# Xiaoming-Zhao/PointNav-VO

Measured on AMD Instinct MI355X. Metric: RGB-D frame-pair VO inferences/s @341x192, higher is better.
Workload: dtype f32

## Files before the change

### pointnav-vo_amd/csrc/conv_x3.hip

```cpp
#include <cmath>
#include <cstdio>
#include <cstdlib>
#include <cstring>

#include "pnvo_internal.h"

namespace pnvo {

typedef float f32x16 __attribute__((ext_vector_type(16)));
typedef float f32x4 __attribute__((ext_vector_type(4)));
typedef float f32x2 __attribute__((ext_vector_type(2)));
typedef __bf16 bf16x8 __attribute__((ext_vector_type(8)));
typedef __bf16 bf16x2 __attribute__((ext_vector_type(2)));
typedef _Float16 f16x8 __attribute__((ext_vector_type(8)));
typedef _Float16 f16x2 __attribute__((ext_vector_type(2)));
typedef unsigned u32x4 __attribute__((ext_vector_type(4)));

namespace {
__device__ __forceinline__ unsigned pack2(float a, float b) {
  const bf16x2 r = __builtin_convertvector(f32x2{a, b}, bf16x2);
  return __builtin_bit_cast(unsigned, r);
}
__device__ __forceinline__ unsigned pack2h(float a, float b) {
  const f16x2 r = __builtin_convertvector(f32x2{a, b}, f16x2);
  return __builtin_bit_cast(unsigned, r);
}
__device__ __forceinline__ float lo_f(unsigned u) { return __builtin_bit_cast(float, u << 16); }
__device__ __forceinline__ float hi_f(unsigned u) { return __builtin_bit_cast(float, u & 0xffff0000u); }
}

constexpr int x3_wpe(int mw, int nw, int np, bool dsf = false) {
  return dsf ? (mw * nw >= 6 ? 1 : (mw * nw >= 2 ? 2 : 3)) : ((np == 2 && mw * nw <= 2) ? 3 : 2);
}

template <int KS, int STRIDE, int MODE, int MW, int NW, int NP, bool DSF = false, bool W8 = false, bool KSW = false>
__global__ __launch_bounds__(W8 ? 512 : 256) __attribute__((amdgpu_waves_per_eu(W8 ? 2 : x3_wpe(MW, NW, NP, DSF), W8 ? 2 : x3_wpe(MW, NW, NP, DSF)))) void conv_x3_kernel(const ConvX3Args p) {
  constexpr int NTH = W8 ? 512 : 256, NWV = NTH / 64;
  constexpr int EMW = KSW ? 1 : MW;
  static_assert(!KSW || (NW == 1 && NP == 2 && KS == 3 && !DSF && !W8), "K split over the waves: float16-piece 3x3 convs, one N-tile");
  static_assert(!DSF || (KS == 3 && STRIDE == 2 && NP == 2 && (MODE == 0 || MODE == 2)), "the downsample rides on a float16-piece 3x3 stride-2 conv");
  extern __shared__ __attribute__((aligned(16))) unsigned char lds[];
  constexpr int PSTEP = KS == 1 ? STRIDE : 1;
  constexpr int CS = KS == 1 ? 1 : STRIDE;
  constexpr int PAD = KS / 2;
  const int lane = threadIdx.x & 63;
  const int wave = __builtin_amdgcn_readfirstlane(threadIdx.x >> 6);

  const int ntiles = p.B * p.tiles_r * p.tiles_c;
  const int chunk = (ntiles + 7) >> 3;
  int bid = (int)(blockIdx.x & 7) * chunk + (int)(blockIdx.x >> 3);
  if (bid >= ntiles) return;
  const int tci = bid % p.tiles_c;
  bid /= p.tiles_c;
  const int tri = bid % p.tiles_r;
  const int n = bid / p.tiles_r;
  const int r0 = tri * p.TR, c0 = tci * p.TC;
  const int hi0 = r0 * STRIDE - PAD, wi0 = c0 * STRIDE - PAD;
  const int mdl = (p.grp_end0 > 0 && n >= p.grp_end0) + (p.grp_end1 > 0 && n >= p.grp_end1);
  const unsigned short *g_wpk = mdl == 0 ? p.wpk : p.wpk_g[mdl - 1];
  const unsigned short *g_ds_wpk = mdl == 0 ? p.ds_wpk : p.ds_wpk_g[mdl - 1];
  const float g_oscale = mdl == 0 ? p.oscale : p.oscale_g[mdl - 1], g_ds_oscale = mdl == 0 ? p.ds_oscale : p.ds_oscale_g[mdl - 1];
  const float *g_gamma = mdl == 0 ? p.gn_gamma : p.gn_gamma_g[mdl - 1], *g_beta = mdl == 0 ? p.gn_beta : p.gn_beta_g[mdl - 1];
  const float *g_ds_gamma = mdl == 0 ? p.ds_gamma : p.ds_gamma_g[mdl - 1], *g_ds_beta = mdl == 0 ? p.ds_beta : p.ds_beta_g[mdl - 1];
  const int PR = p.PR, PC = p.PC, CK = p.CK;
  const int pitch = CK * 2 + 16;
  const int plane = PR * PC * pitch;
  const int npix = p.TR * p.TC;
  const int tab_off = KSW ? max(NP * plane, 4 * MW * 4096) : NP * plane;
  unsigned *qtab = reinterpret_cast<unsigned *>(lds + tab_off);
  unsigned *otab = qtab + p.MT * 32;
  for (int e = (int)threadIdx.x; e < p.MT * 32; e += NTH) {
    const int q = min(e, npix - 1);
    const int tr = q / p.TC, tc = q - tr * p.TC;
    qtab[e] = (unsigned)(((tr * CS) * PC + tc * CS) * pitch);
    const bool ok = e < npix && r0 + tr < p.Ho && c0 + tc < p.Wo;
    otab[e] = (unsigned)((tr * p.Wo + tc) * p.COUTP) | (ok ? 0u : 0x80000000u);
  }

  const int wn = p.wn;
  const int wave_m = wave / wn;
  const int wave_n = (wave & (wn - 1)) + (int)blockIdx.y * wn;
  const int ntt = p.COUTP >> 5, kct = p.CIN >> 4;

  f32x16 acc[MW][NW];
#pragma unroll
  for (int i = 0; i < MW; ++i)
#pragma unroll
    for (int j = 0; j < NW; ++j)
#pragma unroll
      for (int r = 0; r < 16; ++r) acc[i][j][r] = 0.f;
  f32x16 accd[DSF ? MW : 1][DSF ? NW : 1];
  if (DSF) {
#pragma unroll
    for (int i = 0; i < MW; ++i)
#pragma unroll
      for (int j = 0; j < NW; ++j)
#pragma unroll
        for (int r = 0; r < 16; ++r) accd[DSF ? i : 0][DSF ? j : 0][r] = 0.f;
  }

  float in_mul = 1.f, in_div = 1.f;
  const bool in_scaled = NP == 2 && p.in_absmax != nullptr;
  if (in_scaled) {
    unsigned mb = p.in_absmax[(threadIdx.x & 63) * 16];
#pragma unroll
    for (int d = 32; d >= 1; d >>= 1) mb = max(mb, (unsigned)__shfl_xor((int)mb, d));
    const int e = mb != 0u ? (int)((mb >> 23) & 0xffu) - 126 : 14;
    in_mul = __builtin_bit_cast(float, (unsigned)(14 - e + 127) << 23);
    in_div = __builtin_bit_cast(float, (unsigned)(e - 14 + 127) << 23);
  }
  const int G = CK >> 3;
  const int cg = threadIdx.x & (G - 1), pl = threadIdx.x / G, PS = NTH / G;
  const int dr = PS / PC, dc = PS - dr * PC;
  const int nppix = PR * PC;

  unsigned long long c_stage = 0, c_mm = 0, t_0 = __builtin_readcyclecounter(), r_0 = wall_clock64();
  for (int ck0 = 0; ck0 < p.CIN; ck0 += CK) {
    unsigned long long t_a = __builtin_readcyclecounter();
    if (ck0 > 0) __syncthreads();
    {
      f32x4 sc0, sc1, sh0, sh1, rs0, rs1, rt0, rt1;
      const bool res_ss = MODE == 2 && p.res_scale != nullptr;
      auto load_ss = [&]() {
        if (MODE >= 1) {
          const float *ps = p.in_scale + (long)n * p.CIN + ck0 + 8 * cg;
          const float *pt = p.in_shift + (long)n * p.CIN + ck0 + 8 * cg;
          sc0 = *reinterpret_cast<const f32x4 *>(ps);
          sc1 = *reinterpret_cast<const f32x4 *>(ps + 4);
          sh0 = *reinterpret_cast<const f32x4 *>(pt);
          sh1 = *reinterpret_cast<const f32x4 *>(pt + 4);
        }
        if (res_ss) {
          const float *ps = p.res_scale + (long)n * p.CIN + ck0 + 8 * cg;
          const float *pt = p.res_shift + (long)n * p.CIN + ck0 + 8 * cg;
          rs0 = *reinterpret_cast<const f32x4 *>(ps);
          rs1 = *reinterpret_cast<const f32x4 *>(ps + 4);
          rt0 = *reinterpret_cast<const f32x4 *>(pt);
          rt1 = *reinterpret_cast<const f32x4 *>(pt + 4);
        }
      };
      load_ss();
      int pr = pl / PC, pc = pl - pr * PC;
      const long img = ((long)n * p.H * p.W) * p.CIN + ck0 + 8 * cg;
      const float *xb = p.x + img;
      struct Round {
        f32x4 v[2][2], w[2][2];
        unsigned off[2];
        int gofs[2];
        bool ok[2], in[2], own[2];
      };
      auto fetch = [&](int pix, Round &r) {
#pragma unroll
        for (int k = 0; k < 2; ++k) {
          const int hi = hi0 + pr * PSTEP, wi = wi0 + pc * PSTEP;
          r.ok[k] = pix + k * PS < nppix;
          r.in[k] = r.ok[k] && hi >= 0 && hi < p.H && wi >= 0 && wi < p.W;
          r.off[k] = (unsigned)((pr * PC + pc) * pitch + 16 * cg);
          r.v[k][0] = r.v[k][1] = f32x4{0.f, 0.f, 0.f, 0.f};
          if (MODE >= 2) {
            r.own[k] = r.in[k] && p.xout != nullptr && blockIdx.y == 0 && pr >= PAD && pr < PAD + p.TR * CS && pc >= PAD && pc < PAD + p.TC * CS;
            r.gofs[k] = (hi * p.W + wi) * p.CIN;
          }
          if (r.in[k]) {
            const float *src = xb + ((long)hi * p.W + wi) * p.CIN;
            r.v[k][0] = *reinterpret_cast<const f32x4 *>(src);
            r.v[k][1] = *reinterpret_cast<const f32x4 *>(src + 4);
            if (MODE == 2) {
              const float *rsrc = p.res + img + ((long)hi * p.W + wi) * p.CIN;
              r.w[k][0] = *reinterpret_cast<const f32x4 *>(rsrc);
              r.w[k][1] = *reinterpret_cast<const f32x4 *>(rsrc + 4);
            }
          }
          pr += dr;
          pc += dc;
          if (pc >= PC) {
            pc -= PC;
            pr += 1;
          }
        }
      };
      auto split_store = [&](const Round &r) {
#pragma unroll
        for (int k = 0; k < 2; ++k) {
          if (!r.ok[k]) continue;
          float f[8];
#pragma unroll
          for (int e = 0; e < 8; ++e) {
            float t = r.v[k][e >> 2][e & 3];
            if (MODE == 1) {
              const f32x4 &sc = e < 4 ? sc0 : sc1, &sh = e < 4 ? sh0 : sh1;
              t = r.in[k] ? fmaxf(__builtin_fmaf(t, sc[e & 3], sh[e & 3]), 0.f) : 0.f;
            }
            if (MODE == 3) {
              const f32x4 &sc = e < 4 ? sc0 : sc1, &sh = e < 4 ? sh0 : sh1;
              int key = __builtin_bit_cast(int, t);
              key = key >= 0 ? key : key ^ 0x7fffffff;
              t = r.in[k] ? fmaxf(__builtin_fmaf(__builtin_bit_cast(float, key), __builtin_fabsf(sc[e & 3]), sh[e & 3]), 0.f) : 0.f;
            }
            if (MODE == 2) {
              const f32x4 &sc = e < 4 ? sc0 : sc1, &sh = e < 4 ? sh0 : sh1;
              float u = r.w[k][e >> 2][e & 3];
              if (res_ss) u = __builtin_fmaf(u, (e < 4 ? rs0 : rs1)[e & 3], (e < 4 ? rt0 : rt1)[e & 3]);
              t = r.in[k] ? fmaxf(__builtin_fmaf(t, sc[e & 3], sh[e & 3]) + u, 0.f) : 0.f;
            }
            f[e] = t;
          }
          if (MODE >= 2 && r.own[k]) {
            float *dst = p.xout + img + r.gofs[k];
            *reinterpret_cast<f32x4 *>(dst) = f32x4{f[0], f[1], f[2], f[3]};
            *reinterpret_cast<f32x4 *>(dst + 4) = f32x4{f[4], f[5], f[6], f[7]};
          }
          if (NP == 2) {
            if (in_scaled) {
#pragma unroll
              for (int e = 0; e < 8; ++e) f[e] *= in_mul;
            }
            u32x4 o0, o1;
#pragma unroll
            for (int e = 0; e < 4; ++e) {
              const float a = f[2 * e], b = f[2 * e + 1];
              const f16x2 h = __builtin_convertvector(f32x2{a, b}, f16x2);
              o0[e] = __builtin_bit_cast(unsigned, h);
              o1[e] = pack2h(a - (float)h[0], b - (float)h[1]);
            }
            *reinterpret_cast<u32x4 *>(lds + r.off[k]) = o0;
            *reinterpret_cast<u32x4 *>(lds + plane + r.off[k]) = o1;
            continue;
          }
          u32x4 o0, o1, o2;
#pragma unroll
          for (int e = 0; e < 4; ++e) {
            const float a = f[2 * e], b = f[2 * e + 1];
            const unsigned h = pack2(a, b);
            const float ra = a - lo_f(h), rb = b - hi_f(h);
            const unsigned m = pack2(ra, rb);
            o0[e] = h;
            o1[e] = m;
            o2[e] = pack2(ra - lo_f(m), rb - hi_f(m));
          }
          *reinterpret_cast<u32x4 *>(lds + r.off[k]) = o0;
          *reinterpret_cast<u32x4 *>(lds + plane + r.off[k]) = o1;
          *reinterpret_cast<u32x4 *>(lds + 2 * plane + r.off[k]) = o2;
        }
      };
      constexpr bool PIPE = !((MODE == 2 && (MW * NW >= 6 || x3_wpe(MW, NW, NP) == 3 || DSF)) || (DSF && MW * NW == 4));
      if (MW * NW <= 2 && !(MODE == 2 && (x3_wpe(MW, NW, NP) == 3 || DSF))) {
        for (int pix = pl; pix < nppix; pix += 6 * PS) {
          Round r0, r1, r2;
          fetch(pix, r0);
          fetch(pix + 2 * PS, r1);
          fetch(pix + 4 * PS, r2);
          split_store(r0);
          split_store(r1);
          split_store(r2);
        }
      } else if (PIPE) {
        Round cur, nxt;
        fetch(pl, cur);
        for (int pix = pl; pix < nppix; pix += 2 * PS) {
          const bool more = pix + 2 * PS < nppix;
          if (more) fetch(pix + 2 * PS, nxt);
          split_store(cur);
          if (more) cur = nxt;
        }
      } else {
        for (int pix = pl; pix < nppix; pix += 2 * PS) {
          Round cur;
          fetch(pix, cur);
          split_store(cur);
        }
      }
    }
    __syncthreads();
    unsigned long long t_b = __builtin_readcyclecounter();
    c_stage += t_b - t_a;

    unsigned aoff[MW];
#pragma unroll
    for (int i = 0; i < MW; ++i) {
      const int mt = min(KSW ? i : wave_m * MW + i, p.MT - 1);
      aoff[i] = qtab[mt * 32 + (lane & 31)] + (unsigned)((lane >> 5) * 16);
    }
    const int kcc = CK >> 4;
    const int nsteps = KS * KS * kcc;
    const unsigned kstep = (unsigned)ntt * (NP * 1024u);
    const char *wb_n = reinterpret_cast<const char *>(g_wpk) + (long)(ck0 >> 4) * kstep;
    unsigned toff_n = 0;
    int kc_n = 0, kw_n = 0;
    auto advance = [&]() {
      ++kc_n;
      toff_n += 32;
      wb_n += kstep;
      if (kc_n == kcc) {
        kc_n = 0;
        toff_n += (unsigned)(pitch - kcc * 32);
        wb_n += (long)(kct - kcc) * kstep;
        if (++kw_n == KS) {
          kw_n = 0;
          toff_n += (unsigned)((PC - KS) * pitch);
        }
      }
    };
    constexpr bool RING = NP == 2 && KS == 3 && MW * NW <= 2;
    const char *wb_b = wb_n;
    int kc_b = 0;
    auto advanceB = [&]() {
      wb_b += kstep;
      if (++kc_b == kcc) {
        kc_b = 0;
        wb_b += (long)(kct - kcc) * kstep;
      }
    };
    unsigned voff[NW];
#pragma unroll
    for (int j = 0; j < NW; ++j) voff[j] = (unsigned)min(wave_n * NW + j, ntt - 1) * (NP * 1024u) + (unsigned)lane * 16u;
    auto loadBr = [&](u32x4 (*b)[NW]) {
#pragma unroll
      for (int j = 0; j < NW; ++j)
#pragma unroll
        for (int pc = 0; pc < NP; ++pc) b[pc][j] = *reinterpret_cast<const u32x4 *>(wb_b + (size_t)voff[j] + pc * 1024);
    };
    auto loadA = [&](int i, u32x4 (*a)[MW]) {
#pragma unroll
      for (int pc = 0; pc < NP; ++pc) a[pc][i] = *reinterpret_cast<const u32x4 *>(lds + pc * plane + aoff[i] + toff_n);
    };
    auto loadB = [&](u32x4 (*b)[NW]) {
#pragma unroll
      for (int j = 0; j < NW; ++j)
#pragma unroll
        for (int pc = 0; pc < NP; ++pc) b[pc][j] = *reinterpret_cast<const u32x4 *>(wb_n + (size_t)voff[j] + pc * 1024);
    };
    auto step = [&](u32x4 (*a)[MW], const u32x4 (*b)[NW]) {
#pragma unroll
      for (int i = 0; i < MW; ++i) {
#pragma unroll
        for (int j = 0; j < NW; ++j) {
          if (NP == 2) {
            constexpr int TA[3] = {1, 0, 0}, TB[3] = {0, 1, 0};
#pragma unroll
            for (int t = 0; t < 3; ++t)
              acc[i][j] = __builtin_amdgcn_mfma_f32_32x32x16_f16(__builtin_bit_cast(f16x8, a[TA[t]][i]),
                                                                 __builtin_bit_cast(f16x8, b[TB[t]][j]), acc[i][j], 0, 0, 0);
          } else {
            constexpr int TA[6] = {1, 2, 0, 1, 0, 0}, TB[6] = {1, 0, 2, 0, 1, 0};
#pragma unroll
            for (int t = 0; t < 6; ++t)
              acc[i][j] = __builtin_amdgcn_mfma_f32_32x32x16_bf16(__builtin_bit_cast(bf16x8, a[TA[t]][i]),
                                                                  __builtin_bit_cast(bf16x8, b[TB[t]][j]), acc[i][j], 0, 0, 0);
          }
        }
        __builtin_amdgcn_sched_barrier(0);
        loadA(i, a);
        __builtin_amdgcn_sched_barrier(0);
      }
    };
    u32x4 a[NP][MW], b0[NP][NW], b1[NP][NW];
    u32x4 bd0[DSF ? NP : 1][NW], bd1[DSF ? NP : 1][NW];
    auto loadBd = [&](u32x4 (*b)[NW], int kc) {
      const char *wd = reinterpret_cast<const char *>(g_ds_wpk) + (long)((ck0 >> 4) + kc) * kstep;
#pragma unroll
      for (int j = 0; j < NW; ++j)
#pragma unroll
        for (int pc = 0; pc < NP; ++pc) b[pc][j] = *reinterpret_cast<const u32x4 *>(wd + (size_t)voff[j] + pc * 1024);
    };
    if constexpr (KSW) {
      const int s0 = (wave * nsteps) >> 2, s1 = ((wave + 1) * nsteps) >> 2;
      {
        const int tap = s0 / kcc, kc = s0 - tap * kcc, kh = tap / KS, kw = tap - kh * KS;
        kc_n = kc;
        kw_n = kw;
        toff_n = (unsigned)((kh * PC + kw) * pitch + kc * 32);
        wb_n += ((long)tap * kct + kc) * kstep;
        kc_b = kc;
        wb_b = wb_n;
      }
      u32x4 br[3][NP][NW];
      int fb = s0;
      auto fetchB = [&](u32x4 (*bq)[NW]) {
        loadBr(bq);
        if (++fb < s1) advanceB();
      };
      fetchB(br[0]);
      fetchB(br[1]);
#pragma unroll
      for (int i = 0; i < MW; ++i) loadA(i, a);
      if (s0 + 1 < s1) advance();
#pragma unroll 1
      for (int s = s0; s < s1; s += 3) {
#pragma unroll
        for (int u = 0; u < 3; ++u) {
          if (s + u >= s1) break;
          fetchB(br[(u + 2) % 3]);
          __builtin_amdgcn_sched_barrier(0);
          step(a, br[u]);
          if (s + u + 2 < s1) advance();
        }
      }
    } else {
    if (DSF) loadBd(bd0, 0);
    loadB(b0);
#pragma unroll
    for (int i = 0; i < MW; ++i) loadA(i, a);
    advance();
    if (RING) {
      constexpr int R = MW * NW <= 2 ? 6 : 3;
      u32x4 br[R][NP][NW];
#pragma unroll
      for (int pc = 0; pc < NP; ++pc)
#pragma unroll
        for (int j = 0; j < NW; ++j) br[0][pc][j] = b0[pc][j];
#pragma unroll
      for (int q = 1; q < R - 1; ++q) {
        advanceB();
        loadBr(br[q]);
      }
      advanceB();
      constexpr bool A2 = MW * NW <= 2 && !(MODE == 2 && MW * NW == 2 && !DSF) && !(MODE == 2 && DSF && MW * NW == 1);
      u32x4 a1[A2 ? NP : 1][MW];
      if (A2) {
#pragma unroll
        for (int i = 0; i < MW; ++i) loadA(i, a1);
        advance();
      }
#pragma unroll 1
      for (int s = 0; s < nsteps; s += R) {
#pragma unroll
        for (int u = 0; u < R; ++u) {
          loadBr(br[(u + R - 1) % R]);
          if (s + u + R < nsteps) advanceB();
          __builtin_amdgcn_sched_barrier(0);
          if (A2) {
            step((u & 1) ? a1 : a, br[u]);
            if (s + u + 3 < nsteps) advance();
          } else {
            step(a, br[u]);
            if (s + u + 2 < nsteps) advance();
          }
        }
      }
    } else {
#pragma unroll 1
      for (int s = 0; s < nsteps; s += 2) {
        const bool more = s + 2 < nsteps;
        loadB(b1);
        __builtin_amdgcn_sched_barrier(0);
        step(a, b0);
        if (more) advance();
        loadB(b0);
        __builtin_amdgcn_sched_barrier(0);
        step(a, b1);
        if (more) advance();
      }
    }
    }
    if constexpr (DSF) {
      const unsigned tc0 = (unsigned)((PC + 1) * pitch);
      u32x4 ad[NP][MW];
      auto loadAd = [&](int kc) {
#pragma unroll
        for (int i = 0; i < MW; ++i)
#pragma unroll
          for (int pc = 0; pc < NP; ++pc) ad[pc][i] = *reinterpret_cast<const u32x4 *>(lds + pc * plane + aoff[i] + tc0 + (unsigned)kc * 32u);
      };
      auto mm = [&](const u32x4 (*bd)[NW]) {
        constexpr int TA[3] = {1, 0, 0}, TB[3] = {0, 1, 0};
#pragma unroll
        for (int i = 0; i < MW; ++i)
#pragma unroll
          for (int j = 0; j < NW; ++j)
#pragma unroll
            for (int t = 0; t < 3; ++t)
              accd[i][j] = __builtin_amdgcn_mfma_f32_32x32x16_f16(__builtin_bit_cast(f16x8, ad[TA[t]][i]), __builtin_bit_cast(f16x8, bd[TB[t]][j]),
                                                                  accd[i][j], 0, 0, 0);
      };
      if constexpr (MW * NW == 4) {
#pragma unroll 1
        for (int kc = 0; kc < kcc; ++kc) {
          loadAd(kc);
          mm(bd0);
          if (kc + 1 < kcc) loadBd(bd0, kc + 1);
        }
      } else {
#pragma unroll 1
        for (int kc = 0; kc < kcc; kc += 2) {
          loadAd(kc);
          loadBd(bd1, kc + 1);
          mm(bd0);
          loadAd(kc + 1);
          if (kc + 2 < kcc) loadBd(bd0, kc + 2);
          mm(bd1);
        }
      }
    }
    c_mm += __builtin_readcyclecounter() - t_b;
  }
  if constexpr (KSW) {
    __syncthreads();
    float *part = reinterpret_cast<float *>(lds);
#pragma unroll
    for (int i = 0; i < MW; ++i)
#pragma unroll
      for (int r = 0; r < 16; ++r) part[((wave * MW + i) * 16 + r) * 64 + lane] = acc[i][0][r];
    __syncthreads();
    const int mt = min(wave, MW - 1);
#pragma unroll
    for (int r = 0; r < 16; ++r) {
      float v = part[((0 * MW + mt) * 16 + r) * 64 + lane];
#pragma unroll
      for (int w = 1; w < 4; ++w) v += part[((w * MW + mt) * 16 + r) * 64 + lane];
      acc[0][0][r] = v;
    }
    __syncthreads();
  }
  unsigned long long t_e = __builtin_readcyclecounter();

  const int rr16 = lane >> 5;
  const long ybase = (((long)n * p.Ho + r0) * p.Wo + c0) * p.COUTP;
  auto emit = [&](f32x16 (*ac)[NW], float *yout, float *stats, const float *oscale_ptr, float oscale, const float *gamma, const float *beta,
                  float *gscale, float *gshift, float *gmu, float *grstd, bool again) {
    if (NP == 2) {
      const float os = (oscale_ptr != nullptr ? *oscale_ptr : oscale) * in_div;
#pragma unroll
      for (int i = 0; i < EMW; ++i)
#pragma unroll
        for (int j = 0; j < NW; ++j)
#pragma unroll
          for (int r = 0; r < 16; ++r) ac[i][j][r] *= os;
    }
    float t1[NW], t2[NW];
#pragma unroll
    for (int j = 0; j < NW; ++j) t1[j] = t2[j] = 0.f;
#pragma unroll
    for (int i = 0; i < EMW; ++i) {
      const int mt = KSW ? wave : wave_m * MW + i;
      if (mt >= p.MT) continue;
      u32x4 ent[4];
#pragma unroll
      for (int g4 = 0; g4 < 4; ++g4) ent[g4] = *reinterpret_cast<const u32x4 *>(otab + mt * 32 + 8 * g4 + 4 * rr16);
      unsigned flags = 0;
#pragma unroll
      for (int g4 = 0; g4 < 4; ++g4) flags |= ent[g4][0] | ent[g4][1] | ent[g4][2] | ent[g4][3];
      const bool whole = !__any((int)(flags >> 31));
#pragma unroll
      for (int j = 0; j < NW; ++j) {
        const int nt = wave_n * NW + j;
        if (nt >= ntt) continue;
        const int co = nt * 32 + (lane & 31);
        float s1 = 0.f, s2 = 0.f;
        if (whole) {
#pragma unroll
          for (int r = 0; r < 16; ++r) {
            const float v = ac[i][j][r];
            (yout + ybase + co)[ent[r >> 2][r & 3]] = v;
            s1 += v;
            s2 = __builtin_fmaf(v, v, s2);
          }
        } else {
#pragma unroll
          for (int r = 0; r < 16; ++r) {
            const unsigned e = ent[r >> 2][r & 3];
            const bool ok = (int)e >= 0;
            const float v = ok ? ac[i][j][r] : 0.f;
            if (ok) (yout + ybase + co)[e] = v;
            s1 += v;
            s2 = __builtin_fmaf(v, v, s2);
          }
        }
        t1[j] += s1 + __shfl_xor(s1, 32);
        t2[j] += s2 + __shfl_xor(s2, 32);
      }
    }
    if (stats != nullptr) {
      const int rows = NWV / wn;
      float *red = reinterpret_cast<float *>(lds);
      if (rows > 1) {
        __syncthreads();
        if (lane < 32)
// ... 315 lines not shown
#pragma unroll
          for (int r = 0; r < 16; ++r) acc[i][j][r] *= os;
    }
    const int rr16 = lane >> 5;
    const long ybase = (((long)cur.n * p.Ho + cur.r0) * p.Wo + cur.c0) * p.COUTP;
    float t1[NW], t2[NW];
#pragma unroll
    for (int j = 0; j < NW; ++j) t1[j] = t2[j] = 0.f;
#pragma unroll
    for (int i = 0; i < MW; ++i) {
      const int mt = wave_m * MW + i;
      if (mt >= p.MT) continue;
      u32x4 ent[4];
#pragma unroll
      for (int g4 = 0; g4 < 4; ++g4) ent[g4] = *reinterpret_cast<const u32x4 *>(otab + mt * 32 + 8 * g4 + 4 * rr16);
      unsigned flags = 0;
#pragma unroll
      for (int g4 = 0; g4 < 4; ++g4) flags |= ent[g4][0] | ent[g4][1] | ent[g4][2] | ent[g4][3];
      const bool whole = !__any((int)(flags >> 31));
#pragma unroll
      for (int j = 0; j < NW; ++j) {
        const int nt = wave_n * NW + j;
        if (nt >= ntt) continue;
        const int co = nt * 32 + (lane & 31);
        float s1 = 0.f, s2 = 0.f;
        if (whole) {
#pragma unroll
          for (int r = 0; r < 16; ++r) {
            const float x = acc[i][j][r];
            (p.y + ybase + co)[ent[r >> 2][r & 3]] = x;
            s1 += x;
            s2 = __builtin_fmaf(x, x, s2);
          }
        } else {
#pragma unroll
          for (int r = 0; r < 16; ++r) {
            const unsigned e = ent[r >> 2][r & 3];
            const bool ok = (int)e >= 0;
            const float x = ok ? acc[i][j][r] : 0.f;
            if (ok) (p.y + ybase + co)[e] = x;
            s1 += x;
            s2 = __builtin_fmaf(x, x, s2);
          }
        }
        t1[j] += s1 + __shfl_xor(s1, 32);
        t2[j] += s2 + __shfl_xor(s2, 32);
      }
    }
    if (p.stats != nullptr) {
      const int rows = 4 / wn;
      float *red = reinterpret_cast<float *>(lds);
      if (rows > 1) {
        __syncthreads();
        if (lane < 32)
#pragma unroll
          for (int j = 0; j < NW; ++j) *reinterpret_cast<f32x2 *>(red + ((wave * NW + j) * 32 + lane) * 2) = f32x2{t1[j], t2[j]};
        __syncthreads();
      }
      if (wave_m == 0 && lane < 32) {
#pragma unroll
        for (int j = 0; j < NW; ++j) {
          const int nt = wave_n * NW + j;
          if (nt >= ntt) continue;
          float s1 = t1[j], s2 = t2[j];
          for (int w = 1; w < rows; ++w) {
            const f32x2 o = *reinterpret_cast<const f32x2 *>(red + (((w * wn + (wave & (wn - 1))) * NW + j) * 32 + lane) * 2);
            s1 += o[0];
            s2 += o[1];
          }
          float *dst = p.stats + (((long)cur.n * p.slots + cur.tri * p.tiles_c + cur.tci) * p.COUTP + nt * 32 + lane) * 2;
          dst[0] = s1;
          dst[1] = s2;
        }
      }
    }
    if (!nxt.valid) break;
    if (BRES) fetch(nxt);
    __syncthreads();
    cur = nxt;
  }
}

namespace {
template <int KS, int STRIDE, int NP>
hipError_t launch_ks(const ConvX3Args &a, int mode, int mw, int nw, dim3 grid, size_t ldsb, hipStream_t s) {
#define PNVO_X3(MODE_, MW_, NW_)                                                                          \
  if (mode == MODE_ && mw == MW_ && nw == NW_) {                                                          \
    hipLaunchKernelGGL((conv_x3_kernel<KS, STRIDE, MODE_, MW_, NW_, NP>), grid, dim3(256), ldsb, s, a);   \
    return hipGetLastError();                                                                             \
  }
  if constexpr (KS == 3 && STRIDE == 2 && NP == 2) {
    if (a.ds_wpk != nullptr) {
#define PNVO_X3D(MODE_, MW_, NW_)                                                                               \
  if (mode == MODE_ && mw == MW_ && nw == NW_) {                                                                \
    hipLaunchKernelGGL((conv_x3_kernel<KS, STRIDE, MODE_, MW_, NW_, NP, true>), grid, dim3(256), ldsb, s, a);   \
    return hipGetLastError();                                                                                   \
  }
      if (a.w8) {
#define PNVO_X3DW(MODE_)                                                                                                  \
  if (mode == MODE_ && mw == 3 && nw == 1) {                                                                             \
    hipLaunchKernelGGL((conv_x3_kernel<KS, STRIDE, MODE_, 3, 1, NP, true, true>), grid, dim3(512), ldsb, s, a);          \
    return hipGetLastError();                                                                                            \
  }
        PNVO_X3DW(0) PNVO_X3DW(2)
#undef PNVO_X3DW
        return hipErrorInvalidValue;
      }
      PNVO_X3D(0, 1, 1) PNVO_X3D(2, 1, 1) PNVO_X3D(0, 2, 1) PNVO_X3D(2, 2, 1) PNVO_X3D(0, 2, 2) PNVO_X3D(2, 2, 2) PNVO_X3D(0, 3, 2) PNVO_X3D(2, 3, 2)
#undef PNVO_X3D
      return hipErrorInvalidValue;
    }
  }
  PNVO_X3(0, 1, 1) PNVO_X3(1, 1, 1) PNVO_X3(0, 2, 1) PNVO_X3(1, 2, 1) PNVO_X3(0, 2, 2) PNVO_X3(1, 2, 2) PNVO_X3(0, 3, 2) PNVO_X3(1, 3, 2)
  PNVO_X3(2, 1, 1) PNVO_X3(2, 2, 1) PNVO_X3(2, 2, 2) PNVO_X3(2, 3, 2) PNVO_X3(3, 1, 1) PNVO_X3(3, 2, 1) PNVO_X3(3, 2, 2) PNVO_X3(3, 3, 2)

  if (KS == 3 && STRIDE == 1 && NP == 2) {
    PNVO_X3(0, 5, 1) PNVO_X3(1, 5, 1) PNVO_X3(2, 5, 1) PNVO_X3(3, 5, 1)
    if constexpr (KS == 3 && STRIDE == 1 && NP == 2) if (a.ksw) {
#define PNVO_X3K(MODE_, MW_)                                                                                             \
  if (mode == MODE_ && mw == MW_ && nw == 1) {                                                                          \
    hipLaunchKernelGGL((conv_x3_kernel<KS, STRIDE, MODE_, MW_, 1, NP, false, false, true>), grid, dim3(256), ldsb, s, a); \
    return hipGetLastError();                                                                                           \
  }
      PNVO_X3K(0, 3) PNVO_X3K(1, 3) PNVO_X3K(2, 3) PNVO_X3K(0, 4) PNVO_X3K(1, 4) PNVO_X3K(2, 4)
#undef PNVO_X3K
      return hipErrorInvalidValue;
    }
  }
  if constexpr (KS == 3 && NP == 2) if (a.w8) {
#define PNVO_X3W(MODE_)                                                                                                  \
  if (mode == MODE_ && mw == 3 && nw == 1) {                                                                            \
  hipLaunchKernelGGL((conv_x3_kernel<KS, STRIDE, MODE_, 3, 1, NP, false, true>), grid, dim3(512), ldsb, s, a);        \
  return hipGetLastError();                                                                                           \
  }
    PNVO_X3W(0) PNVO_X3W(1) PNVO_X3W(2) PNVO_X3W(3)
#undef PNVO_X3W
    return hipErrorInvalidValue;
  }
#undef PNVO_X3
  return hipErrorInvalidValue;
}
}

namespace {
bool conv_x3_plan_impl(ConvX3Args &a, int ks, int stride, int *mw, int *nw, size_t *lds_bytes, bool fine);
long plan_wgs(const ConvX3Args &a, int nw) {
  const int ntt = a.COUTP / 32;
  return (long)a.B * a.tiles_r * a.tiles_c * ((ntt + a.wn * nw - 1) / (a.wn * nw));
}
}

bool conv_x3_plan(ConvX3Args &a, int ks, int stride, int *mw, int *nw, size_t *lds_bytes) {
  ConvX3Args reg = a;
  int rmw = 0, rnw = 0;
  size_t rlds = 0;
  const int force0 = a.force;
  reg.force = 1;
  const bool reg_ok = conv_x3_plan_impl(reg, ks, stride, &rmw, &rnw, &rlds, false);
  const long reg_wgs = reg_ok ? plan_wgs(reg, rnw) : 0;
  const int ntt = a.COUTP / 32;
  if (a.fine && a.np == 2 && ntt >= 2 && (!reg_ok || reg_wgs < 224)) {
    ConvX3Args f = a;
    int fmw = 0, fnw = 0;
    size_t flds = 0;
    f.force = 1;
    if (conv_x3_plan_impl(f, ks, stride, &fmw, &fnw, &flds, true)) {
      const long fw = plan_wgs(f, fnw);
      if (fw > reg_wgs && (fw >= 48 || force0)) {
        f.force = force0;
        a = f;
        *mw = fmw;
        *nw = fnw;
        *lds_bytes = flds;
        return true;
      }
    }
  }
  return conv_x3_plan_impl(a, ks, stride, mw, nw, lds_bytes, false);
}

namespace {
bool conv_x3_plan_impl(ConvX3Args &a, int ks, int stride, int *mw, int *nw, size_t *lds_bytes, bool fine) {
  if (a.CIN % 32 || a.COUTP % 32 || a.COUTP > 1024 || a.CIN > 1024) return false;
  if (!((ks == 3 && (stride == 1 || stride == 2)) || (ks == 1 && stride == 2))) return false;
  a.w8 = 0;
  a.ksw = 0;
  const int ntt = a.COUTP / 32;
  int TR, TC;
  if (stride == 2 && ks == 3) {
    TC = a.Wo >= 32 ? 16 : a.Wo;
    const int pc = 2 * TC + 1;
    TR = (324 / pc - 1) / 2;
    if (TR < 1) return false;
    if (TR > a.Ho) TR = a.Ho;
    while (TR > 1 && TR * TC > (ntt == 2 ? 64 : (ntt == 4 ? 128 : 96))) --TR;
  } else if (ntt == 1 && stride == 1 && ks == 3 && a.CIN > 32 && a.np == 2 && a.Wo < 32 && a.Ho * a.Wo <= 128) {
    TC = a.Wo;
    TR = a.Ho;
  } else if (ntt == 1) {
    if (stride != 1 || ks != 3 || a.CIN != 32) return false;
    TC = a.Wo >= 16 ? 16 : a.Wo;
    TR = 256 / TC;
    while (TR > 1 && (TR + 2) * (TC + 2) > 324) --TR;
    if (TR > a.Ho) TR = a.Ho;
    if (TR * TC <= 96) return false;
  } else if (a.strip && !fine && a.np == 2 && stride == 1 && ks == 3 && ntt == 4 && a.Wo >= 16 && a.Ho >= 8) {
    const int ncol = (a.Wo + 21) / 22;
    TC = (a.Wo + ncol - 1) / ncol;
    TR = 288 / TC;
    if (TR > a.Ho) TR = a.Ho;
    const int nrow = (a.Ho + TR - 1) / TR;
    TR = (a.Ho + nrow - 1) / nrow;
  } else if (a.Wo >= 32) {
    TR = 8;
    TC = 16;
  } else {
    TC = a.Wo;
    int target = ntt == 4 ? 192 : (ntt >= 8 ? 96 : 128);
    if (fine && a.ksw_ok && ks == 3 && stride == 1 && a.np == 2 && a.CIN >= 128) target = 96;
    TR = target / TC;
    if (TR < 1) TR = 1;
    if (TR > a.Ho) TR = a.Ho;
  }
  a.TR = TR;
  a.TC = TC;
  a.tiles_r = (a.Ho + TR - 1) / TR;
  a.tiles_c = (a.Wo + TC - 1) / TC;
  a.MT = (TR * TC + 31) / 32;
  const int cs = ks == 1 ? 1 : stride;
  a.PR = (TR - 1) * cs + ks;
  a.PC = (TC - 1) * cs + ks;
  const bool strip = a.strip && !fine && a.np == 2 && stride == 1 && ks == 3 && ntt == 4 && a.Wo >= 16 && a.Ho >= 8 && a.MT > 6;
  if (fine) {
    if (a.MT > 8) return false;
    a.wn = 1;
    *mw = (a.MT + 3) / 4;
    *nw = 1;
    if (a.ksw_ok && (a.MT == 3 || a.MT == 4) && ks == 3 && stride == 1 && a.np == 2 && a.CIN >= 128) {
      a.ksw = 1;
      *mw = a.MT;
    }
  } else if (strip) {
    a.wn = 2;
    *mw = (a.MT + 1) / 2;
    *nw = 1;
    if (*mw > 5) return false;
    if (*mw < 5) *mw = 5;
  } else if (ntt == 1) {
    a.wn = 1;
    *mw = a.CIN > 32 ? 1 : 2;
    *nw = 1;
    if (a.ksw_ok && a.CIN >= 128 && (a.MT == 3 || a.MT == 4) && ks == 3 && stride == 1 && a.np == 2) {
      a.ksw = 1;
      *mw = a.MT;
    }
  } else if (ntt == 2) {
    a.wn = 2;
    *mw = a.MT > 2 ? 2 : 1;
    *nw = 1;
  } else if (ntt == 4) {
    a.wn = 2;
    *mw = a.MT > 4 ? 3 : 2;
    *nw = 2;
  } else {
    a.wn = 4;
    *mw = a.MT > 2 ? 3 : 2;
    *nw = 2;
    const long ntiles = (long)a.B * a.tiles_r * a.tiles_c;
    if (ntiles < 200 && a.MT <= 4) {
      a.wn = 2;
      *mw = 2;
    }
    if (a.w8_ok && !fine && ntiles >= 200 && a.MT == 3 && ntt == 8 && a.np == 2 && ks == 3) {
      a.w8 = 1;
      a.wn = 8;
      *mw = 3;
      *nw = 1;
    }
  }
  if (!a.ksw && ((a.w8 ? 8 : 4) / a.wn) * *mw < a.MT) return false;
  const size_t np = a.np == 2 ? 2 : 3;
  int ck = 32;
  while (ck < 256 && a.CIN % (2 * ck) == 0) ck *= 2;
  const size_t cap = (size_t)72 * 1024;
  while (ck > 32 && np * a.PR * a.PC * (ck * 2 + 16) > cap) ck /= 2;
  if (np * a.PR * a.PC * (ck * 2 + 16) > cap + 4096) return false;
  if (a.CIN % ck) return false;
  a.CK = ck;
  {
    const bool force = a.force != 0;
    const long wgs = (long)a.B * a.tiles_r * a.tiles_c * ((ntt + a.wn * *nw - 1) / (a.wn * *nw));
    if (wgs < (a.np == 2 ? 112 : 192) && !force) return false;
  }
  a.slots = a.tiles_r * a.tiles_c;
  *lds_bytes = np * a.PR * a.PC * (ck * 2 + 16) + (size_t)a.MT * 32 * 4 * 2;
  if (a.ksw) *lds_bytes = std::max(np * a.PR * a.PC * (ck * 2 + 16), (size_t)4 * a.MT * 4096) + (size_t)a.MT * 32 * 4 * 2;
  return true;
}
}

bool conv_x3_persistent(const ConvX3Args &a, int ks, int stride, int mode, int mw, int nw) {
  const long ntiles = (long)a.B * a.tiles_r * a.tiles_c;
  const int ntt = a.COUTP / 32, pwgs = a.persist_wgs;
  const bool bres = ntt == 1 && a.CIN == 32 && nw == 1 && (mode == 0 || mode == 1);
  return a.np == 2 && ks == 3 && stride == 1 && bres && mw * nw <= 2 && a.CK == a.CIN && pwgs >= 8 &&
         (long)a.PR * a.PC * (a.CK / 8) <= 6 * 256 && ntiles >= 2L * pwgs;
}

hipError_t launch_conv_x3(const ConvX3Args &a0, int ks, int stride, int mode, int mw, int nw, size_t lds_bytes, hipStream_t s) {
  ConvX3Args a = a0;
  static unsigned long long *prof = nullptr;
  static const bool want = std::getenv("PNVO_X3_PROF") != nullptr;
  if (want && !prof) {
    (void)hipMalloc((void **)&prof, 512);
    (void)hipMemset(prof, 0, 512);
  }
  a.prof = prof;
  struct Dump {
    const ConvX3Args &a; int mw, nw; hipStream_t s; unsigned long long *prof;
    ~Dump() {
      static int calls = 0;
      if (!prof || ++calls > 40) return;
      unsigned long long h[64];
      (void)hipStreamSynchronize(s);
      (void)hipMemcpy(h, prof, 512, hipMemcpyDeviceToHost);
      std::fprintf(stderr, "[pnvo] conv_x3 B %d %dx%d cin %d cout %d tile %dx%d MT %d CK %d (%d,%d) wn %d: wave0 stage %llu mfma %llu epi %llu total %llu "
                           "(100MHz ticks %llu) | wave3 stage %llu mfma %llu epi %llu total %llu\n", a.B, a.Ho, a.Wo, a.CIN, a.COUTP, a.TR, a.TC,
                   a.MT, a.CK, mw, nw, a.wn, h[0], h[1], h[2], h[3], h[4], h[24], h[25], h[26], h[27]);
    }
  } dump{a, mw, nw, s, prof};
  const long ntiles = (long)a.B * a.tiles_r * a.tiles_c;
  const int ntt = a.COUTP / 32, per_wg = a.wn * nw;
  dim3 grid((unsigned)(((ntiles + 7) / 8) * 8), (unsigned)((ntt + per_wg - 1) / per_wg), 1u);
  const int pwgs = a.persist_wgs;
  if (conv_x3_persistent(a, ks, stride, mode, mw, nw)) {
    const bool bres = true;
    dim3 pg((unsigned)(pwgs & ~7), grid.y, 1u);
    if (bres) pg.x = (unsigned)(((pwgs / 3) * 2) & ~7);
#define PNVO_X3P(MODE_, MW_, NW_)                                                                        \
  if (mode == MODE_ && mw == MW_ && nw == NW_) {                                                         \
    hipLaunchKernelGGL((conv_x3p_kernel<MODE_, MW_, NW_, true>), pg, dim3(256), lds_bytes, s, a);       \
    return hipGetLastError();                                                                            \
  }
    PNVO_X3P(0, 1, 1) PNVO_X3P(1, 1, 1) PNVO_X3P(0, 2, 1) PNVO_X3P(1, 2, 1)
#undef PNVO_X3P
  }
  if (a.np == 2) {
    if (ks == 3 && stride == 1) return launch_ks<3, 1, 2>(a, mode, mw, nw, grid, lds_bytes, s);
    if (ks == 3 && stride == 2) return launch_ks<3, 2, 2>(a, mode, mw, nw, grid, lds_bytes, s);
    if (ks == 1 && stride == 2) return launch_ks<1, 2, 2>(a, mode, mw, nw, grid, lds_bytes, s);
    return hipErrorInvalidValue;
  }
  if (ks == 3 && stride == 1) return launch_ks<3, 1, 3>(a, mode, mw, nw, grid, lds_bytes, s);
  if (ks == 3 && stride == 2) return launch_ks<3, 2, 3>(a, mode, mw, nw, grid, lds_bytes, s);
  if (ks == 1 && stride == 2) return launch_ks<1, 2, 3>(a, mode, mw, nw, grid, lds_bytes, s);
  return hipErrorInvalidValue;
}

void pack_conv_x3_weight(const float *oihw, int cout, int cin, int cinp, int coutp, int kh_, int kw_, unsigned short *out) {
  const int T = kh_ * kw_, kct = cinp / 16, ntt = coutp / 32;
  auto bf = [](float f) {
    unsigned u;
    std::memcpy(&u, &f, 4);
    if ((u & 0x7f800000u) == 0x7f800000u) return (unsigned short)(u >> 16);
    u += 0x7fffu + ((u >> 16) & 1u);
    return (unsigned short)(u >> 16);
  };
  auto tof = [](unsigned short h) {
    const unsigned u = (unsigned)h << 16;
    float f;
    std::memcpy(&f, &u, 4);
    return f;
  };
  for (int tap = 0; tap < T; ++tap)
    for (int kc = 0; kc < kct; ++kc)
      for (int nt = 0; nt < ntt; ++nt)
        for (int ln = 0; ln < 64; ++ln)
          for (int j = 0; j < 8; ++j) {
// ... 147 lines not shown
```

Measured before the change: 115,700.

## Double-buffer LDS chunk staging in eight-wave conv kernel to overlap loads with MFMA

The eight-wave conv_x3 kernel now keeps two LDS staging sets. The next input-channel chunk is fetched into registers during the matrix loop and stored to the alternate buffer afterwards, which removes one barrier per chunk and hides global-load latency. It also enables the eight-wave variant for strip tiles with five M-tiles per wave, raises the dynamic LDS limit, and adds a fit check. The cost is double the LDS footprint, more registers for the prefetch, and unconditional loads that may read clamped addresses.

```diff
diff --git a/pointnav-vo_amd/csrc/conv_x3.hip b/pointnav-vo_amd/csrc/conv_x3.hip
--- a/pointnav-vo_amd/csrc/conv_x3.hip
+++ b/pointnav-vo_amd/csrc/conv_x3.hip
@@ -2,6 +2,7 @@
 #include <cstdio>
 #include <cstdlib>
 #include <cstring>
+#include <type_traits>
 
 #include "pnvo_internal.h"
 
@@ -33,12 +34,24 @@
   return dsf ? (mw * nw >= 6 ? 1 : (mw * nw >= 2 ? 2 : 3)) : ((np == 2 && mw * nw <= 2) ? 3 : 2);
 }
 
+constexpr int x3_pl_pixels(int mw, bool dsf) { return (dsf || mw == 5) ? 3 : 4; }
+
+template <int N>
+struct X3Round {
+  static constexpr int n = N;
+  f32x4 v[N][2], w[N][2];
+  unsigned off[N];
+  int gofs[N];
+  bool ok[N], in[N], own[N];
+};
+
 template <int KS, int STRIDE, int MODE, int MW, int NW, int NP, bool DSF = false, bool W8 = false, bool KSW = false>
 __global__ __launch_bounds__(W8 ? 512 : 256) __attribute__((amdgpu_waves_per_eu(W8 ? 2 : x3_wpe(MW, NW, NP, DSF), W8 ? 2 : x3_wpe(MW, NW, NP, DSF)))) void conv_x3_kernel(const ConvX3Args p) {
   constexpr int NTH = W8 ? 512 : 256, NWV = NTH / 64;
   constexpr int EMW = KSW ? 1 : MW;
   static_assert(!KSW || (NW == 1 && NP == 2 && KS == 3 && !DSF && !W8), "K split over the waves: float16-piece 3x3 convs, one N-tile");
   static_assert(!DSF || (KS == 3 && STRIDE == 2 && NP == 2 && (MODE == 0 || MODE == 2)), "the downsample rides on a float16-piece 3x3 stride-2 conv");
+  static_assert(!W8 || (KS == 3 && NP == 2 && MW * NW >= 3 && !KSW), "eight waves (pipelined chunk loop): float16-piece 3x3 convs");
   extern __shared__ __attribute__((aligned(16))) unsigned char lds[];
   constexpr int PSTEP = KS == 1 ? STRIDE : 1;
   constexpr int CS = KS == 1 ? 1 : STRIDE;
@@ -65,8 +78,9 @@
   const int PR = p.PR, PC = p.PC, CK = p.CK;
   const int pitch = CK * 2 + 16;
   const int plane = PR * PC * pitch;
+  const unsigned setb = (unsigned)(NP * plane);
   const int npix = p.TR * p.TC;
-  const int tab_off = KSW ? max(NP * plane, 4 * MW * 4096) : NP * plane;
+  const int tab_off = KSW ? max(NP * plane, 4 * MW * 4096) : (W8 ? 2 : 1) * NP * plane;
   unsigned *qtab = reinterpret_cast<unsigned *>(lds + tab_off);
   unsigned *otab = qtab + p.MT * 32;
   for (int e = (int)threadIdx.x; e < p.MT * 32; e += NTH) {
@@ -115,43 +129,43 @@
   const int nppix = PR * PC;
 
   unsigned long long c_stage = 0, c_mm = 0, t_0 = __builtin_readcyclecounter(), r_0 = wall_clock64();
-  for (int ck0 = 0; ck0 < p.CIN; ck0 += CK) {
+  unsigned st_off = 0;
+  for (int ck0 = W8 ? -CK : 0; ck0 < p.CIN; ck0 += CK) {
     unsigned long long t_a = __builtin_readcyclecounter();
-    if (ck0 > 0) __syncthreads();
-    {
+    if (!W8 && ck0 > 0) __syncthreads();
+    const bool stg = !W8 || ck0 + CK < p.CIN;
+    const int cks = W8 ? (stg ? ck0 + CK : 0) : ck0;
+    const unsigned st_base = W8 ? st_off : 0u, mm_base = W8 ? setb - st_off : 0u;
+    constexpr int NPX = x3_pl_pixels(MW, DSF);
       f32x4 sc0, sc1, sh0, sh1, rs0, rs1, rt0, rt1;
       const bool res_ss = MODE == 2 && p.res_scale != nullptr;
       auto load_ss = [&]() {
         if (MODE >= 1) {
-          const float *ps = p.in_scale + (long)n * p.CIN + ck0 + 8 * cg;
-          const float *pt = p.in_shift + (long)n * p.CIN + ck0 + 8 * cg;
+          const float *ps = p.in_scale + (long)n * p.CIN + cks + 8 * cg;
+          const float *pt = p.in_shift + (long)n * p.CIN + cks + 8 * cg;
           sc0 = *reinterpret_cast<const f32x4 *>(ps);
           sc1 = *reinterpret_cast<const f32x4 *>(ps + 4);
           sh0 = *reinterpret_cast<const f32x4 *>(pt);
           sh1 = *reinterpret_cast<const f32x4 *>(pt + 4);
         }
         if (res_ss) {
-          const float *ps = p.res_scale + (long)n * p.CIN + ck0 + 8 * cg;
-          const float *pt = p.res_shift + (long)n * p.CIN + ck0 + 8 * cg;
+          const float *ps = p.res_scale + (long)n * p.CIN + cks + 8 * cg;
+          const float *pt = p.res_shift + (long)n * p.CIN + cks + 8 * cg;
           rs0 = *reinterpret_cast<const f32x4 *>(ps);
           rs1 = *reinterpret_cast<const f32x4 *>(ps + 4);
           rt0 = *reinterpret_cast<const f32x4 *>(pt);
           rt1 = *reinterpret_cast<const f32x4 *>(pt + 4);
         }
       };
-      load_ss();
+      if (!W8) load_ss();
       int pr = pl / PC, pc = pl - pr * PC;
-      const long img = ((long)n * p.H * p.W) * p.CIN + ck0 + 8 * cg;
+      const long img = ((long)n * p.H * p.W) * p.CIN + cks + 8 * cg;
       const float *xb = p.x + img;
-      struct Round {
-        f32x4 v[2][2], w[2][2];
-        unsigned off[2];
-        int gofs[2];
-        bool ok[2], in[2], own[2];
-      };
-      auto fetch = [&](int pix, Round &r) {
-#pragma unroll
-        for (int k = 0; k < 2; ++k) {
+      using Round = X3Round<2>;
+      auto fetch = [&](int pix, auto &r) {
+        constexpr int RN = std::remove_reference_t<decltype(r)>::n;
+#pragma unroll
+        for (int k = 0; k < RN; ++k) {
           const int hi = hi0 + pr * PSTEP, wi = wi0 + pc * PSTEP;
           r.ok[k] = pix + k * PS < nppix;
           r.in[k] = r.ok[k] && hi >= 0 && hi < p.H && wi >= 0 && wi < p.W;
@@ -161,7 +175,15 @@
             r.own[k] = r.in[k] && p.xout != nullptr && blockIdx.y == 0 && pr >= PAD && pr < PAD + p.TR * CS && pc >= PAD && pc < PAD + p.TC * CS;
             r.gofs[k] = (hi * p.W + wi) * p.CIN;
           }
-          if (r.in[k]) {
+          if constexpr (W8) {
+            const long po = r.in[k] && stg ? ((long)hi * p.W + wi) * p.CIN : 0L;
+            r.v[k][0] = *reinterpret_cast<const f32x4 *>(xb + po);
+            r.v[k][1] = *reinterpret_cast<const f32x4 *>(xb + po + 4);
+            if (MODE == 2) {
+              r.w[k][0] = *reinterpret_cast<const f32x4 *>(p.res + img + po);
+              r.w[k][1] = *reinterpret_cast<const f32x4 *>(p.res + img + po + 4);
+            }
+          } else if (r.in[k]) {
             const float *src = xb + ((long)hi * p.W + wi) * p.CIN;
             r.v[k][0] = *reinterpret_cast<const f32x4 *>(src);
             r.v[k][1] = *reinterpret_cast<const f32x4 *>(src + 4);
@@ -179,14 +201,16 @@
           }
         }
       };
-      auto split_store = [&](const Round &r) {
-#pragma unroll
-        for (int k = 0; k < 2; ++k) {
+      auto split_store = [&](const auto &r) {
+        constexpr int RN = std::remove_reference_t<decltype(r)>::n;
+#pragma unroll
+        for (int k = 0; k < RN; ++k) {
           if (!r.ok[k]) continue;
           float f[8];
 #pragma unroll
           for (int e = 0; e < 8; ++e) {
             float t = r.v[k][e >> 2][e & 3];
+            if (W8 && MODE == 0) t = r.in[k] ? t : 0.f;
             if (MODE == 1) {
               const f32x4 &sc = e < 4 ? sc0 : sc1, &sh = e < 4 ? sh0 : sh1;
               t = r.in[k] ? fmaxf(__builtin_fmaf(t, sc[e & 3], sh[e & 3]), 0.f) : 0.f;
@@ -223,8 +247,8 @@
               o0[e] = __builtin_bit_cast(unsigned, h);
               o1[e] = pack2h(a - (float)h[0], b - (float)h[1]);
             }
-            *reinterpret_cast<u32x4 *>(lds + r.off[k]) = o0;
-            *reinterpret_cast<u32x4 *>(lds + plane + r.off[k]) = o1;
+            *reinterpret_cast<u32x4 *>(lds + st_base + r.off[k]) = o0;
+            *reinterpret_cast<u32x4 *>(lds + st_base + plane + r.off[k]) = o1;
             continue;
           }
           u32x4 o0, o1, o2;
@@ -244,7 +268,18 @@
         }
       };
       constexpr bool PIPE = !((MODE == 2 && (MW * NW >= 6 || x3_wpe(MW, NW, NP) == 3 || DSF)) || (DSF && MW * NW == 4));
-      if (MW * NW <= 2 && !(MODE == 2 && (x3_wpe(MW, NW, NP) == 3 || DSF))) {
+      X3Round<W8 ? NPX : 1> nx;
+      if constexpr (W8) {
+        if (ck0 < 0) {
+          load_ss();
+          fetch(pl, nx);
+          split_store(nx);
+          st_off = setb - st_off;
+          __syncthreads();
+          c_stage += __builtin_readcyclecounter() - t_a;
+          continue;
+        }
+      } else if (MW * NW <= 2 && !(MODE == 2 && (x3_wpe(MW, NW, NP) == 3 || DSF))) {
         for (int pix = pl; pix < nppix; pix += 6 * PS) {
           Round r0, r1, r2;
           fetch(pix, r0);
@@ -270,8 +305,7 @@
           split_store(cur);
         }
       }
-    }
-    __syncthreads();
+    if (!W8) __syncthreads();
     unsigned long long t_b = __builtin_readcyclecounter();
     c_stage += t_b - t_a;
 
@@ -279,7 +313,7 @@
 #pragma unroll
     for (int i = 0; i < MW; ++i) {
       const int mt = min(KSW ? i : wave_m * MW + i, p.MT - 1);
-      aoff[i] = qtab[mt * 32 + (lane & 31)] + (unsigned)((lane >> 5) * 16);
+      aoff[i] = qtab[mt * 32 + (lane & 31)] + (unsigned)((lane >> 5) * 16) + mm_base;
     }
     const int kcc = CK >> 4;
     const int nsteps = KS * KS * kcc;
@@ -301,7 +335,7 @@
         }
       }
     };
-    constexpr bool RING = NP == 2 && KS == 3 && MW * NW <= 2;
+    constexpr bool RING = NP == 2 && KS == 3 && (MW * NW <= 2 || W8);
     const char *wb_b = wb_n;
     int kc_b = 0;
     auto advanceB = [&]() {
@@ -403,7 +437,7 @@
     for (int i = 0; i < MW; ++i) loadA(i, a);
     advance();
     if (RING) {
-      constexpr int R = MW * NW <= 2 ? 6 : 3;
+      constexpr int R = (MW * NW <= 2 || MW == 3) ? 6 : 3;
       u32x4 br[R][NP][NW];
 #pragma unroll
       for (int pc = 0; pc < NP; ++pc)
@@ -422,8 +456,7 @@
         for (int i = 0; i < MW; ++i) loadA(i, a1);
         advance();
       }
-#pragma unroll 1
-      for (int s = 0; s < nsteps; s += R) {
+      auto period = [&](const int s) {
 #pragma unroll
         for (int u = 0; u < R; ++u) {
           loadBr(br[(u + R - 1) % R]);
@@ -437,6 +470,17 @@
             if (s + u + 2 < nsteps) advance();
           }
         }
+      };
+      if constexpr (W8) {
+        load_ss();
+        fetch(pl, nx);
+        __builtin_amdgcn_sched_barrier(0);
+        period(0);
+#pragma unroll 1
+        for (int s = R; s < nsteps; s += R) period(s);
+      } else {
+#pragma unroll 1
+        for (int s = 0; s < nsteps; s += R) period(s);
       }
     } else {
 #pragma unroll 1
@@ -492,7 +536,18 @@
         }
       }
     }
-    c_mm += __builtin_readcyclecounter() - t_b;
+    if constexpr (W8) {
+      const unsigned long long t_c = __builtin_readcyclecounter();
+      c_mm += t_c - t_b;
+      if (stg) {
+        split_store(nx);
+        st_off = setb - st_off;
+        __syncthreads();
+      }
+      c_stage += __builtin_readcyclecounter() - t_c;
+    } else {
+      c_mm += __builtin_readcyclecounter() - t_b;
+    }
   }
   if constexpr (KSW) {
     __syncthreads();
@@ -974,6 +1029,23 @@
 }
 
 namespace {
+template <auto KERNEL>
+hipError_t x3_allow_lds() {
+  static std::mutex mu;
+  static unsigned long long seen = 0;
+  if (!pnvo_first_launch_on_device(mu, seen)) return hipSuccess;
+  return hipFuncSetAttribute(reinterpret_cast<const void *>(KERNEL), hipFuncAttributeMaxDynamicSharedMemorySize, 160 * 1024);
+}
+int x3_chunk(const ConvX3Args &a) {
+  const size_t np = a.np == 2 ? 2 : 3;
+  int ck = 32;
+  while (ck < 256 && a.CIN % (2 * ck) == 0) ck *= 2;
+  const size_t cap = (size_t)72 * 1024;
+  while (ck > 32 && np * a.PR * a.PC * (ck * 2 + 16) > cap) ck /= 2;
+  return ck;
+}
+bool x3_w8_fits(const ConvX3Args &a, int mw, bool dsf) { return a.PR * a.PC <= x3_pl_pixels(mw, dsf) * (512 / (x3_chunk(a) / 8)); }
+
 template <int KS, int STRIDE, int NP>
 hipError_t launch_ks(const ConvX3Args &a, int mode, int mw, int nw, dim3 grid, size_t ldsb, hipStream_t s) {
 #define PNVO_X3(MODE_, MW_, NW_)                                                                          \
@@ -991,7 +1063,9 @@
       if (a.w8) {
 #define PNVO_X3DW(MODE_)                                                                                                  \
   if (mode == MODE_ && mw == 3 && nw == 1) {                                                                             \
-    hipLaunchKernelGGL((conv_x3_kernel<KS, STRIDE, MODE_, 3, 1, NP, true, true>), grid, dim3(512), ldsb, s, a);          \
+    constexpr auto kern = conv_x3_kernel<KS, STRIDE, MODE_, 3, 1, NP, true, true>;                          \
+    if (hipError_t e = x3_allow_lds<kern>(); e != hipSuccess) return e;                                                  \
+    hipLaunchKernelGGL(kern, grid, dim3(512), ldsb, s, a);                                                               \
     return hipGetLastError();                                                                                            \
   }
         PNVO_X3DW(0) PNVO_X3DW(2)
@@ -1002,6 +1076,19 @@
 #undef PNVO_X3D
       return hipErrorInvalidValue;
     }
+  }
+  if constexpr (KS == 3 && NP == 2) if (a.w8) {
+#define PNVO_X3W(MODE_, MW_)                                                                                             \
+  if (mode == MODE_ && mw == MW_ && nw == 1) {                                                                          \
+    constexpr auto kern = conv_x3_kernel<KS, STRIDE, MODE_, MW_, 1, NP, false, true>;                      \
+    if (hipError_t e = x3_allow_lds<kern>(); e != hipSuccess) return e;                                                 \
+    hipLaunchKernelGGL(kern, grid, dim3(512), ldsb, s, a);                                                              \
+    return hipGetLastError();                                                                                           \
+  }
+    PNVO_X3W(0, 3) PNVO_X3W(1, 3) PNVO_X3W(2, 3) PNVO_X3W(3, 3)
+    if constexpr (STRIDE == 1) { PNVO_X3W(0, 5) PNVO_X3W(1, 5) PNVO_X3W(2, 5) PNVO_X3W(3, 5) }
+#undef PNVO_X3W
+    return hipErrorInvalidValue;
   }
   PNVO_X3(0, 1, 1) PNVO_X3(1, 1, 1) PNVO_X3(0, 2, 1) PNVO_X3(1, 2, 1) PNVO_X3(0, 2, 2) PNVO_X3(1, 2, 2) PNVO_X3(0, 3, 2) PNVO_X3(1, 3, 2)
   PNVO_X3(2, 1, 1) PNVO_X3(2, 2, 1) PNVO_X3(2, 2, 2) PNVO_X3(2, 3, 2) PNVO_X3(3, 1, 1) PNVO_X3(3, 2, 1) PNVO_X3(3, 2, 2) PNVO_X3(3, 3, 2)
@@ -1018,16 +1105,6 @@
 #undef PNVO_X3K
       return hipErrorInvalidValue;
     }
-  }
-  if constexpr (KS == 3 && NP == 2) if (a.w8) {
-#define PNVO_X3W(MODE_)                                                                                                  \
-  if (mode == MODE_ && mw == 3 && nw == 1) {                                                                            \
-  hipLaunchKernelGGL((conv_x3_kernel<KS, STRIDE, MODE_, 3, 1, NP, false, true>), grid, dim3(512), ldsb, s, a);        \
-  return hipGetLastError();                                                                                           \
-  }
-    PNVO_X3W(0) PNVO_X3W(1) PNVO_X3W(2) PNVO_X3W(3)
-#undef PNVO_X3W
-    return hipErrorInvalidValue;
   }
 #undef PNVO_X3
   return hipErrorInvalidValue;
@@ -1138,6 +1215,10 @@
     *nw = 1;
     if (*mw > 5) return false;
     if (*mw < 5) *mw = 5;
+    if (a.w8_ok && (long)a.B * a.tiles_r * a.tiles_c >= 200 && a.tiles_r * a.tiles_c == 1 && a.MT == 9 && x3_w8_fits(a, 5, false)) {
+      a.w8 = 1;
+      a.wn = 4;
+    }
   } else if (ntt == 1) {
     a.wn = 1;
     *mw = a.CIN > 32 ? 1 : 2;
@@ -1163,7 +1244,7 @@
       a.wn = 2;
       *mw = 2;
     }
-    if (a.w8_ok && !fine && ntiles >= 200 && a.MT == 3 && ntt == 8 && a.np == 2 && ks == 3) {
+    if (a.w8_ok && !fine && ntiles >= 200 && a.MT == 3 && ntt == 8 && a.np == 2 && ks == 3 && x3_w8_fits(a, 3, stride == 2)) {
       a.w8 = 1;
       a.wn = 8;
       *mw = 3;
@@ -1172,11 +1253,8 @@
   }
   if (!a.ksw && ((a.w8 ? 8 : 4) / a.wn) * *mw < a.MT) return false;
   const size_t np = a.np == 2 ? 2 : 3;
-  int ck = 32;
-  while (ck < 256 && a.CIN % (2 * ck) == 0) ck *= 2;
-  const size_t cap = (size_t)72 * 1024;
-  while (ck > 32 && np * a.PR * a.PC * (ck * 2 + 16) > cap) ck /= 2;
-  if (np * a.PR * a.PC * (ck * 2 + 16) > cap + 4096) return false;
+  const int ck = x3_chunk(a);
+  if (np * a.PR * a.PC * (ck * 2 + 16) > (size_t)72 * 1024 + 4096) return false;
   if (a.CIN % ck) return false;
   a.CK = ck;
   {
@@ -1185,7 +1263,8 @@
     if (wgs < (a.np == 2 ? 112 : 192) && !force) return false;
   }
   a.slots = a.tiles_r * a.tiles_c;
-  *lds_bytes = np * a.PR * a.PC * (ck * 2 + 16) + (size_t)a.MT * 32 * 4 * 2;
+  const size_t sets = a.w8 ? 2 : 1;
+  *lds_bytes = sets * np * a.PR * a.PC * (ck * 2 + 16) + (size_t)a.MT * 32 * 4 * 2;
   if (a.ksw) *lds_bytes = std::max(np * a.PR * a.PC * (ck * 2 + 16), (size_t)4 * a.MT * 4096) + (size_t)a.MT * 32 * 4 * 2;
   return true;
 }
```

Result: slower. 99500, median of 2 (-14.0%).
